# uta-smile/Adaptive-Graph-Convolutional-Network

Measured on NVIDIA B200. Metric: sgc_ll_train_graphs_per_s, higher is better.
Workload: dtype f32

## Files before the change

adaptive-graph-convolutional-network_b200/csrc/agcn_capi.cu:

```cuda
#include <algorithm>

#include "agcn_internal.cuh"

using namespace agcn;

namespace {

inline size_t align256(size_t x) { return (x + 255) & ~(size_t)255; }

int node_gemm_tn(const GemmTNArgs& t, cudaStream_t st) {
  if (tc_gemm_tn_supported(t)) return tc_gemm_tn(t, st);
  return gemm_tn(t, st);
}

int node_gemm(const GemmArgs& g, float* tc_scratch, cudaStream_t st, bool presplit = false) {
  if (tc_gemm_supported(g)) {
    if (!presplit) {
      int rc = tc_gemm_split_b(g, tc_scratch, st);
      if (rc) return rc;
    }
    return tc_gemm(g, tc_scratch, st);
  }
  return gemm_rows(g, st);
}
// ... 5 lines not shown
  g.A0 = X; g.lda0 = d->F;
  g.A1 = T; g.lda1 = d->F; g.sliceA1 = (int64_t)R * d->F;
  g.B = weight; g.ldb = d->K * d->Fo; g.sliceB = d->Fo;
  g.C = Y; g.ldc = d->Fo;
  g.bias = bias; g.act = d->activation;
  return g;
}

GemmArgs g_gemm_args(const agcn_sgcll_desc* d, int R, const float* dYp, const float* weight, float* C) {
  GemmArgs g;
  g.M = R; g.N = d->F; g.Kd = d->Fo; g.Z = d->K;
  g.A0 = dYp; g.lda0 = d->Fo;
  g.B = weight; g.ldb = d->K * d->Fo; g.sliceB = d->Fo; g.transB = 1;
  g.C = C; g.ldc = d->F; g.sliceC = (int64_t)R * d->F;
  return g;
}

struct Carver {
  char* base;
  size_t off = 0;
  explicit Carver(void* p) : base(reinterpret_cast<char*>(p)) {}
  float* take(size_t floats) {
    float* r = base ? reinterpret_cast<float*>(base + off) : nullptr;
    off += align256(floats * sizeof(float));
    return r;
  }
};

struct Modes {
  bool shortcut, paper, reslap, full, need_dL;
};

Modes modes_of(const agcn_sgcll_desc* d) {
  Modes m;
  m.shortcut = literal_shortcut(d->variant, d->laplacian_mode);
  m.paper = d->laplacian_mode == AGCN_LAP_PAPER;
  m.reslap = d->variant == AGCN_VARIANT_SGC_LL_RESLAP;
  m.full = m.paper && d->metric_grad == AGCN_METRIC_GRAD_FULL;
  m.need_dL = !m.shortcut;
  return m;
}

struct Saved {
  float *T, *Lall, *dist, *dis, *stats, *XW, *tcG, *ftG;
  size_t bytes;
};

Saved carve_saved(const agcn_sgcll_desc* d, const agcn_plan* p, void* base) {
  const Modes m = modes_of(d);
  Carver c(base);
  Saved s{};
  s.T = c.take((size_t)(d->K > 1 ? d->K - 1 : 0) * p->R * d->F);
  s.Lall = m.shortcut ? nullptr : c.take((size_t)p->LL);
  s.dist = m.paper ? c.take((size_t)p->LL) : nullptr;
  s.dis = m.paper ? c.take((size_t)p->R) : nullptr;
  s.stats = m.shortcut ? nullptr : c.take((size_t)4 * p->B);
  s.XW = m.full ? c.take((size_t)p->R * d->F) : nullptr;
  s.tcG = c.take(tc_gemm_scratch_floats(d->F, d->Fo, 1, d->K));
  s.ftG = c.take(fused_w_floats(d->F, d->Fo, d->K));
  s.bytes = c.off;
  return s;
}

inline int64_t dl_stride(const agcn_plan* p) { return (p->LL + 63) & ~(int64_t)63; }
inline int dl_parts(const agcn_sgcll_desc* d, const agcn_plan* p) {
  if (d->K < 2) return 1;
  int parts = std::min(8, (d->F + 31) / 32);
  while (parts > 1 && (int64_t)parts * dl_stride(p) * 4 > ((int64_t)1 << 30)) --parts;
  return std::max(1, parts);
}

struct Work {
  float *XW, *dYp, *G, *V, *tn_part, *act_part, *dL, *dXW, *dalpha_part, *dbeta_part, *tcY, *tcM, *big, *ftY;
  size_t bytes;
};

Work carve_work(const agcn_sgcll_desc* d, const agcn_plan* p, void* base) {
  const Modes m = modes_of(d);
  Carver c(base);
  Work w{};
  w.XW = c.take((size_t)p->R * d->F);
  w.dYp = c.take((size_t)p->R * d->Fo);
  w.G = c.take((size_t)d->K * p->R * d->F);
  w.V = c.take((size_t)(d->K > 1 ? d->K - 1 : 0) * p->R * d->Fo);
  size_t tn = gemm_tn_partial_floats((int)p->R, d->F, d->Fo, d->K);
  if (m.full) tn = std::max(tn, gemm_tn_partial_floats((int)p->R, d->F, d->F, 1));
  {
    GemmTNArgs t;
    t.M = (int)p->R; t.Kd = d->F; t.N = d->Fo; t.S = d->K;
    tn = std::max(tn, tc_gemm_tn_partial_floats(t));
    t.N = d->F; t.S = 1;
    tn = std::max(tn, tc_gemm_tn_partial_floats(t));
  }
  w.tn_part = c.take(tn);
  w.act_part = c.take(act_bwd_partial_floats(p->R, d->Fo));
  w.dL = m.need_dL ? c.take((size_t)dl_parts(d, p) * dl_stride(p)) : nullptr;
  w.dXW = m.full ? c.take((size_t)p->R * d->F) : nullptr;
  w.dalpha_part = c.take((size_t)p->B);
  w.dbeta_part = c.take((size_t)p->B);
  w.tcY = c.take(tc_gemm_scratch_floats(d->Fo, d->F, d->K, 1));
  w.tcM = c.take(tc_gemm_scratch_floats(d->F, d->F, 1, 1));
  w.big = c.take(big_work_floats(p, m.full));
  w.ftY = c.take(fused_w_floats(d->Fo, d->F, d->K));
  w.bytes = c.off;
  return w;
}

int check_desc(const agcn_sgcll_desc* d, const agcn_plan* p) {
  AGCN_REQUIRE(d && p, "null desc or plan");
  AGCN_REQUIRE(d->F >= 1 && d->Fo >= 1 && d->K >= 1, "F, Fo, K must be >= 1");
  AGCN_REQUIRE(d->variant == AGCN_VARIANT_SGC_LL || d->variant == AGCN_VARIANT_SGC_LL_RESLAP, "unknown variant");
  AGCN_REQUIRE(d->laplacian_mode == AGCN_LAP_REFERENCE_LITERAL || d->laplacian_mode == AGCN_LAP_PAPER,
               "unknown laplacian_mode");
  AGCN_REQUIRE(d->metric_grad == AGCN_METRIC_GRAD_REFERENCE || d->metric_grad == AGCN_METRIC_GRAD_FULL,
               "unknown metric_grad");
  AGCN_REQUIRE(d->activation == AGCN_ACT_LINEAR || d->activation == AGCN_ACT_RELU, "unknown activation");
  AGCN_REQUIRE(p->R < (1ll << 31) / std::max(d->F, d->Fo), "batch too large for 32-bit row indexing");
  return AGCN_OK;
}

}

namespace {

int padded_features(const agcn_sgcll_desc* d, const agcn_plan* p) {
  const int F = d->F;
  if (F < 33 || F % 32 == 0) return F;
  if (!literal_shortcut(d->variant, d->laplacian_mode)) return F;
  if (d->flags & (AGCN_OUT_RES_L | AGCN_OUT_RES_W | AGCN_OUT_L_ALL)) return F;
  const int Fp = (F + 31) & ~31;
  if (!fused_fwd_supported(p, Fp, d->Fo, d->K)) return F;
  return Fp;
}

struct PadSaved {
  float *Xp, *Wp;
  void* inner;
  size_t bytes;
};
PadSaved carve_pad_saved(const agcn_sgcll_desc* d2, const agcn_plan* p, void* base) {
  Carver c(base);
  PadSaved s{};
  s.Xp = c.take((size_t)p->R * d2->F);
  s.Wp = c.take((size_t)d2->F * d2->K * d2->Fo);
  s.inner = base ? reinterpret_cast<char*>(base) + c.off : nullptr;
  s.bytes = c.off + carve_saved(d2, p, nullptr).bytes + 256;
  return s;
}
struct PadWork {
  float *dXp, *dWp, *dMp;
  void* inner;
  size_t inner_bytes, bytes;
};
PadWork carve_pad_work(const agcn_sgcll_desc* d2, const agcn_plan* p, void* base) {
  Carver c(base);
  PadWork w{};
  w.dXp = c.take((size_t)p->R * d2->F);
  w.dWp = c.take((size_t)d2->F * d2->K * d2->Fo);
  w.dMp = c.take((size_t)d2->F * d2->F);
  w.inner = base ? reinterpret_cast<char*>(base) + c.off : nullptr;
  w.inner_bytes = carve_work(d2, p, nullptr).bytes + 256;
  w.bytes = c.off + w.inner_bytes;
  return w;
}

__global__ void pad_cols_kernel(const float* __restrict__ src, int Fs, float* __restrict__ dst, int Fd, long long rows) {
  const long long total = rows * Fd;
// ... 162 lines not shown
    AGCN_CUDA(cudaStreamWaitEvent(plan->side, plan->ev_side_fork, 0));
    if (fuse_f && (rc = fused_fwd_prep(d_weight, F, Fo, K, wk.ftY, plan->side))) return rc;
    if (y_tc && (rc = tc_gemm_split_b(gy, wk.tcY, plan->side))) return rc;
    if (fuse_b && (rc = fused_bwd_prep(d_weight, F, Fo, K, sv.ftG, plan->side))) return rc;
    if (g_tc && (rc = tc_gemm_split_b(gg, sv.tcG, plan->side))) return rc;
    AGCN_CUDA(cudaEventRecord(plan->ev_side_join, plan->side));
  }
  if (need_W) {
    GemmArgs g;
    g.M = R; g.N = F; g.Kd = F;
    g.A0 = d_X; g.lda0 = F;
    g.B = d_M_L; g.ldb = F;
    g.C = XW; g.ldc = F;
    if ((rc = node_gemm(g, wk.tcM, st))) return rc;
  }
  GraphArgs ga;
  ga.plan = plan; ga.F = F; ga.K = K;
  ga.variant = desc->variant; ga.lap_mode = desc->laplacian_mode; ga.metric_full = m.full;
  ga.X = d_X; ga.XW = XW; ga.Lint = d_Lint; ga.Lprev = m.reslap ? d_Lprev : nullptr;
  ga.alpha = d_alpha; ga.beta = d_beta;
  ga.T = sv.T;
  if (need_build) {
    ga.Lall = m.shortcut ? nullptr : sv.Lall;
    ga.Lall_out = want_Lall ? d_Lall : nullptr;
    ga.resL = want_resL ? d_resL : nullptr;
    ga.resW = want_resW ? d_resW : nullptr;
    ga.dist = sv.dist; ga.dis = sv.dis; ga.stats = sv.stats;
    ga.big_work = wk.big;
    if ((rc = graph_build_laplacian(ga, need_W, st))) return rc;
  }
  ga.Lall = m.shortcut ? nullptr : sv.Lall;
  if (fuse_f) {
    const float* Lf = m.shortcut ? d_Lint : sv.Lall;
    const int ident = m.shortcut ? 1 : 0;
    const bool other = cheb_tiles_has_mid(plan) || plan->large_tiles > 0;
    if (other) {
      AGCN_CUDA(cudaEventRecord(plan->ev_big_fork, st));
      AGCN_CUDA(cudaStreamWaitEvent(plan->big, plan->ev_big_fork, 0));
    }
    if ((rc = cheb_tiles_forward(plan, d_X, Lf, ident, F, K, sv.T, st, plan->big))) return rc;
    if (plan->large_tiles > 0 && (rc = graph_chebyshev_fwd(ga, plan->big, AGCN_SMALL_MAX))) return rc;
    if (other) {
      AGCN_CUDA(cudaEventRecord(plan->ev_big_join, plan->big));
      AGCN_CUDA(cudaStreamWaitEvent(st, plan->ev_big_join, 0));
    }
    AGCN_CUDA(cudaStreamWaitEvent(st, plan->ev_side_join, 0));
    return pre_forward(plan, -1, 0, d_X, sv.T, wk.ftY, d_bias, desc->activation, F, Fo, K, d_Y, st);
  }
  if ((rc = graph_chebyshev_fwd(ga, st))) return rc;
  if (y_tc || g_tc || fuse_b) AGCN_CUDA(cudaStreamWaitEvent(st, plan->ev_side_join, 0));
  if ((rc = node_gemm(gy, wk.tcY, st, true))) return rc;
  return AGCN_OK;
}

int backward_impl(const agcn_sgcll_desc* desc, const agcn_plan* plan, const float* d_X, const float* d_Lint,
                  const float* d_Lprev, const float* d_M_L, const float* d_weight, const float* d_alpha,
                  const float* d_beta, const float* d_Y, const float* d_dY, const float* d_dLall_in, const void* d_saved,
                  float* d_dX, float* d_dM_L, float* d_dweight, float* d_dbias, float* d_dalpha, float* d_dbeta,
                  float* d_dLprev, void* d_work, size_t work_bytes, void* stream) {
  int rc = check_desc(desc, plan);
  if (rc) return rc;
  AGCN_REQUIRE(d_X && d_Lint && d_M_L && d_weight && d_alpha && d_Y && d_dY && d_saved && d_work,
               "backward: null input pointer");
  AGCN_REQUIRE(d_dM_L && d_dweight && d_dbias && d_dalpha, "backward: null output pointer");
  const Modes m = modes_of(desc);
  AGCN_REQUIRE(!m.reslap || (d_beta && d_dbeta), "backward: beta / dbeta required for SGC_LL_Reslap");
  cudaStream_t st = (cudaStream_t)stream;
  if ((rc = plan_use(plan, st))) return rc;
  Saved sv = carve_saved(desc, plan, const_cast<void*>(d_saved));
  Work wk = carve_work(desc, plan, d_work);
  if (wk.bytes > work_bytes) {
    set_error("backward: workspace too small");
    return AGCN_ERR_WORKSPACE;
  }
  const int F = desc->F, Fo = desc->Fo, K = desc->K;
  const int R = (int)plan->R;
  const bool has_prev = m.reslap && d_Lprev;

  const bool fuse_b = (desc->flags & AGCN_SAVE_FOR_BACKWARD) && !m.need_dL && d_dX != nullptr &&
                      fused_bwd_supported(plan, F, Fo, K);
  const bool vfirst = fuse_b && plan->large_tiles == 0;
  const bool need_G = !fuse_b && (d_dX != nullptr || (m.need_dL && K >= 2));
  const float* dYp = (desc->activation == AGCN_ACT_RELU) ? wk.dYp : d_dY;
  const bool act_on_side = !vfirst && (fuse_b || (!need_G && !m.need_dL));
  if (!act_on_side && (rc = act_bwd_partials(d_dY, d_Y, wk.dYp, wk.act_part, R, Fo, desc->activation, st))) return rc;
  AGCN_CUDA(cudaEventRecord(plan->ev_side_fork, st));
  AGCN_CUDA(cudaStreamWaitEvent(plan->side, plan->ev_side_fork, 0));
  if (act_on_side && (rc = act_bwd_partials(d_dY, d_Y, wk.dYp, wk.act_part, R, Fo, desc->activation, plan->side)))
    return rc;
  if ((rc = act_bwd_reduce(wk.act_part, d_dbias, R, Fo, plan->side))) return rc;
  float* dXbuf = d_dX ? d_dX : wk.G;
  AGCN_REQUIRE(d_dX || !m.full, "backward: d_dX is required with metric_grad = full");
  if (need_G) {
    GemmArgs g = g_gemm_args(desc, R, dYp, d_weight, (K == 1) ? d_dX : wk.G);
    GemmArgs probe = g_gemm_args(desc, R, d_Y, d_weight, wk.G);
    const bool presplit = (desc->flags & AGCN_SAVE_FOR_BACKWARD) && tc_gemm_supported(probe);
    if ((rc = node_gemm(g, sv.tcG, st, presplit))) return rc;
  }
  GraphArgs ga;
  ga.plan = plan; ga.F = F; ga.K = K;
  ga.variant = desc->variant; ga.lap_mode = desc->laplacian_mode; ga.metric_full = m.full;
  ga.X = d_X; ga.XW = sv.XW; ga.Lint = d_Lint; ga.Lprev = has_prev ? d_Lprev : nullptr;
  ga.alpha = d_alpha; ga.beta = d_beta;
  ga.T = sv.T; ga.Lall = m.shortcut ? nullptr : sv.Lall;
  ga.dist = sv.dist; ga.dis = sv.dis; ga.stats = sv.stats;
  ga.G = wk.G; ga.dLall_in = d_dLall_in; ga.dX = dXbuf; ga.dL = wk.dL;
  ga.dl_parts = (m.need_dL && K >= 2) ? dl_parts(desc, plan) : 1;
  ga.dl_stride = dl_stride(plan);
  ga.dLprev = has_prev ? d_dLprev : nullptr;
  ga.dXW = wk.dXW; ga.dalpha_part = wk.dalpha_part; ga.dbeta_part = m.reslap ? wk.dbeta_part : nullptr;
  ga.big_work = wk.big;
  {
    GemmTNArgs t;
    t.M = R; t.Kd = F; t.N = Fo; t.S = K;
    t.A0 = d_X; t.lda0 = F;
    t.A1 = sv.T; t.lda1 = F; t.sliceA1 = (int64_t)R * F;
    t.D = dYp; t.ldd = Fo;
    t.out = d_dweight; t.partial = wk.tn_part;
    if ((rc = node_gemm_tn(t, plan->side))) return rc;
  }
  AGCN_CUDA(cudaEventRecord(plan->ev_side_join, plan->side));
  if (vfirst) {
    const float* Lf = m.shortcut ? d_Lint : sv.Lall;
    const int ident = m.shortcut ? 1 : 0;
    const bool other = cheb_tiles_has_mid(plan);
    if (other) {
      AGCN_CUDA(cudaEventRecord(plan->ev_big_fork, st));
      AGCN_CUDA(cudaStreamWaitEvent(plan->big, plan->ev_big_fork, 0));
    }
    if ((rc = cheb_tiles_forward(plan, dYp, Lf, ident, Fo, K, wk.V, st, plan->big, 1))) return rc;
    if (other) {
      AGCN_CUDA(cudaEventRecord(plan->ev_big_join, plan->big));
      AGCN_CUDA(cudaStreamWaitEvent(st, plan->ev_big_join, 0));
    }
    if ((rc = pre_forward(plan, -1, 0, dYp, wk.V, sv.ftG, nullptr, AGCN_ACT_LINEAR, Fo, F, K, d_dX, st))) return rc;
  } else if (fuse_b) {
    const float* Lf = m.shortcut ? d_Lint : sv.Lall;
    const int ident = m.shortcut ? 1 : 0;
    if ((rc = pre_backward(plan, -1, 0, d_dY, desc->activation == AGCN_ACT_RELU ? d_Y : nullptr, sv.ftG, F, Fo, K, wk.G, st)))
      return rc;
    const bool other = cheb_tiles_has_mid(plan) || plan->large_tiles > 0;
    if (other) {
      AGCN_CUDA(cudaEventRecord(plan->ev_big_fork, st));
      AGCN_CUDA(cudaStreamWaitEvent(plan->big, plan->ev_big_fork, 0));
    }
    if ((rc = cheb_tiles_backward(plan, wk.G, Lf, ident, F, K, d_dX, st, plan->big))) return rc;
    if (plan->large_tiles > 0 && (rc = graph_recurrence_bwd(ga, false, plan->big, AGCN_SMALL_MAX))) return rc;
    if (other) {
      AGCN_CUDA(cudaEventRecord(plan->ev_big_join, plan->big));
      AGCN_CUDA(cudaStreamWaitEvent(st, plan->ev_big_join, 0));
    }
  } else if (K >= 2) {
    if (need_G && (rc = graph_recurrence_bwd(ga, m.need_dL, st))) return rc;
  } else if (m.need_dL) {
    if (d_dLall_in)
      AGCN_CUDA(cudaMemcpyAsync(wk.dL, d_dLall_in, (size_t)plan->LL * sizeof(float), cudaMemcpyDeviceToDevice, st));
    else
      AGCN_CUDA(cudaMemsetAsync(wk.dL, 0, (size_t)plan->LL * sizeof(float), st));
  }
  AGCN_CUDA(cudaStreamWaitEvent(st, plan->ev_side_join, 0));
  if (m.need_dL) {
    if ((rc = graph_laplacian_bwd(ga, st))) return rc;
    if ((rc = reduce_scalar_parts(wk.dalpha_part, plan->B, d_dalpha, st))) return rc;
    if (m.reslap) {
      if ((rc = reduce_scalar_parts(wk.dbeta_part, plan->B, d_dbeta, st))) return rc;
    }
  } else {
    if ((rc = zero_async(d_dalpha, 1, st))) return rc;
  }
  if (m.full) {
    GemmTNArgs t;
    t.M = R; t.Kd = F; t.N = F; t.S = 1;
    t.A0 = d_X; t.lda0 = F;
    t.D = wk.dXW; t.ldd = F;
    t.out = d_dM_L; t.partial = wk.tn_part;
    if ((rc = node_gemm_tn(t, st))) return rc;
    GemmArgs g;
    g.M = R; g.N = F; g.Kd = F;
    g.A0 = wk.dXW; g.lda0 = F;
    g.B = d_M_L; g.ldb = F; g.transB = 1;
    g.C = d_dX; g.ldc = F; g.accumulate = 1;
    if ((rc = node_gemm(g, wk.tcM, st))) return rc;
  } else {
    if ((rc = zero_async(d_dM_L, (size_t)F * F, st))) return rc;
  }
  return AGCN_OK;
}

}

extern "C" {

size_t agcn_gemm_tn_scratch_bytes(int32_t M, int32_t Kd, int32_t N, int32_t S) {
  GemmTNArgs t;
  t.M = M; t.Kd = Kd; t.N = N; t.S = S;
  return 4 * std::max(gemm_tn_partial_floats(M, Kd, N, S), tc_gemm_tn_partial_floats(t)) + 256;
}

int agcn_gemm_tn(const float* d_A0, const float* d_A1, const float* d_D, float* d_out, int32_t M, int32_t Kd,
                 int32_t N, int32_t S, void* d_scratch, int32_t use_tensor_cores, void* stream) {
  AGCN_REQUIRE(d_A0 && d_D && d_out && d_scratch && M >= 1 && Kd >= 1 && N >= 1 && S >= 1, "gemm_tn: bad arguments");
  GemmTNArgs t;
  t.M = M; t.Kd = Kd; t.N = N; t.S = S;
  t.A0 = d_A0; t.lda0 = Kd;
  t.A1 = d_A1; t.lda1 = Kd; t.sliceA1 = (int64_t)M * Kd;
  t.D = d_D; t.ldd = N;
  t.out = d_out; t.partial = reinterpret_cast<float*>(d_scratch);
  if (use_tensor_cores) {
    if (!tc_gemm_tn_supported(t)) {
      set_error("gemm_tn: shape not supported by the tensor-core kernel");
      return AGCN_ERR_INVALID;
    }
    return tc_gemm_tn(t, (cudaStream_t)stream);
  }
  return gemm_tn(t, (cudaStream_t)stream);
}

size_t agcn_node_gemm_scratch_bytes(int32_t N, int32_t Kd) { return 4 * tc_gemm_scratch_floats(N, Kd, 1, 1) + 256; }

int agcn_node_gemm(const float* d_A, int32_t lda, const float* d_B, int32_t ldb, int32_t transB, float* d_C, int32_t ldc,
                   int32_t M, int32_t N, int32_t Kd, const float* d_bias, const float* d_scale, int32_t accumulate,
                   int32_t activation, void* d_scratch, void* stream) {
  AGCN_REQUIRE(d_A && d_B && d_C && d_scratch && M >= 1 && N >= 1 && Kd >= 1, "node_gemm: bad arguments");
  AGCN_REQUIRE(activation == AGCN_ACT_LINEAR || activation == AGCN_ACT_RELU, "node_gemm: unknown activation");
  GemmArgs g;
  g.M = M; g.N = N; g.Kd = Kd;
  g.A0 = d_A; g.lda0 = lda;
  g.B = d_B; g.ldb = ldb; g.transB = transB;
  g.C = d_C; g.ldc = ldc;
  g.bias = d_bias; g.scale = d_scale; g.accumulate = accumulate; g.act = activation;
  return node_gemm(g, reinterpret_cast<float*>(d_scratch), (cudaStream_t)stream);
}

int agcn_fused_profile(int enable) {
  fused_profile_enable(enable);
  return AGCN_OK;
}
int agcn_fused_profile_read(float* ms_sum, int* launches) { return fused_profile_read(ms_sum, launches); }

int agcn_fused_debug_set(void* d_buf) {
  fused_debug_set(d_buf);
  return AGCN_OK;
}

int agcn_sgcll_host_scratch_bytes(const agcn_sgcll_desc* desc, const agcn_plan* plan, size_t* bytes) {
  AGCN_REQUIRE(desc && plan && bytes, "null pointer");
  size_t saved = 0, work = 0;
  agcn_sgcll_workspace_bytes(desc, plan, &saved, &work);
  const size_t B = plan->B, N = plan->Nmax;
  size_t total = 0;
  total += align256(B * N * desc->F * 4) + align256(B * N * N * 4) + align256(B * N * desc->Fo * 4);
  total += align256((size_t)plan->R * desc->F * 4) + align256((size_t)plan->LL * 4) +
           align256((size_t)plan->R * desc->Fo * 4);
  total += align256(saved) + align256(work);
  *bytes = total;
  return AGCN_OK;
}

int agcn_sgcll_forward_host(const agcn_sgcll_desc* desc, const agcn_plan* plan, const float* h_X_padded,
                            const float* h_L_padded, const float* d_M_L, const float* d_weight, const float* d_bias,
                            const float* d_alpha, float* h_Y_padded, void* d_scratch, size_t scratch_bytes,
                            void* stream) {
  int rc = check_desc(desc, plan);
  if (rc) return rc;
  AGCN_REQUIRE(h_X_padded && h_L_padded && h_Y_padded && d_scratch, "forward_host: null pointer");
  AGCN_REQUIRE(desc->variant == AGCN_VARIANT_SGC_LL, "forward_host: SGC_LL only");
  AGCN_REQUIRE((desc->flags & (AGCN_OUT_RES_L | AGCN_OUT_RES_W | AGCN_OUT_L_ALL)) == 0,
// ... 54 lines not shown
```

adaptive-graph-convolutional-network_b200/csrc/agcn_cheb_tile.cu:

```cuda
#include <algorithm>
#include <mutex>

#include "agcn_internal.cuh"

namespace agcn {
namespace ct {

constexpr int CH = 32;
constexpr int CPITCH = 144;

__device__ __forceinline__ uint32_t smem_u32(const void* p) { return (uint32_t)__cvta_generic_to_shared(p); }
__device__ __forceinline__ float4 lds128(uint32_t a) {
  float4 v;
  asm volatile("ld.shared.v4.f32 {%0,%1,%2,%3}, [%4];\n" : "=f"(v.x), "=f"(v.y), "=f"(v.z), "=f"(v.w) : "r"(a) : "memory");
  return v;
}
__device__ __forceinline__ float lds32(uint32_t a) {
  float v;
  asm volatile("ld.shared.f32 %0, [%1];\n" : "=f"(v) : "r"(a) : "memory");
  return v;
}
__device__ __forceinline__ void sts128(uint32_t a, float4 v) {
  asm volatile("st.shared.v4.f32 [%0], {%1,%2,%3,%4};\n" ::"r"(a), "f"(v.x), "f"(v.y), "f"(v.z), "f"(v.w) : "memory");
}
__device__ __forceinline__ void sts32(uint32_t a, float v) {
  asm volatile("st.shared.f32 [%0], %1;\n" ::"r"(a), "f"(v) : "memory");
}
__device__ __forceinline__ void cp_async4(uint32_t sdst, const float* gsrc) {
  asm volatile("cp.async.ca.shared.global [%0], [%1], 4;\n" ::"r"(sdst), "l"(gsrc) : "memory");
}
__device__ __forceinline__ void cp_async16(uint32_t sdst, const float* gsrc) {
  asm volatile("cp.async.cg.shared.global [%0], [%1], 16;\n" ::"r"(sdst), "l"(gsrc) : "memory");
}
__device__ __forceinline__ void cp_async_commit() { asm volatile("cp.async.commit_group;\n" ::: "memory"); }
__device__ __forceinline__ void cp_async_wait_all() { asm volatile("cp.async.wait_group 0;\n" ::: "memory"); }

struct CtArgs {
  const int4* tile_graphs;
  const int32_t* tile_gstart;
  const int32_t* order;
  const int32_t* n_nodes;
  const int32_t* node_off;
  const int64_t* lap_off;
  int order_start;
  int chunks;
  int cpc;
  int groups;
  int rows;
  int lfloats;
  const float* L;
  int add_identity;
  int transL;
  int F, K;
  const float* X;
  float* T;
  long long tslice;
  const float* G;
  long long gslice;
  float* dX;
  unsigned long long* dbg;
};

#define CT_STAMP(slot)                                                                  \
  do {                                                                                  \
    if (p.dbg && threadIdx.x == 0) {                                                    \
      unsigned long long t__;                                                           \
      asm volatile("mov.u64 %0, %%globaltimer;\n" : "=l"(t__));                         \
      p.dbg[(long long)blockIdx.x * 128 + (slot)] = t__;                                \
    }                                                                                   \
  } while (0)

struct Row {
  int grow;
  int n;
  int r0;
  int lbase;
  int i;
  int pitch;
};

__device__ __forceinline__ void copy_matrix(const float* __restrict__ src, uint32_t dst, int n, int pitch) {
  const int warp = threadIdx.x >> 5, lane = threadIdx.x & 31, nw = blockDim.x >> 5;
  for (int i = warp; i < n; i += nw) {
    const float* srow = src + (long long)i * n;
    const uint32_t drow = dst + 4 * (i * pitch);
    for (int j = lane; j < n; j += 32) cp_async4(drow + 4 * j, srow + j);
  }
}

template <bool TILE>
__device__ __forceinline__ Row prologue(const CtArgs& p, int tile, int r, uint32_t s_glist, uint32_t sL) {
  Row t;
  t.grow = -1; t.n = 0; t.r0 = 0; t.lbase = 0; t.i = 0; t.pitch = 1;
  const int tid = threadIdx.x, nthreads = blockDim.x;
  if (TILE) {
    if (tid < 32) {
      int gs = 0, ge = 0;
      if (tid == 0) {
        gs = __ldg(p.tile_gstart + tile);
        ge = __ldg(p.tile_gstart + tile + 1);
      }
      gs = __shfl_sync(0xffffffffu, gs, 0);
      ge = __shfl_sync(0xffffffffu, ge, 0);
      const int ng2 = 2 * (ge - gs);
      for (int e = tid; e < ng2; e += 32) {
        const int4 v = __ldg(p.tile_graphs + 2 * gs + e);
        asm volatile("st.shared.v4.s32 [%0], {%1,%2,%3,%4};\n" ::"r"(s_glist + 16 * e), "r"(v.x), "r"(v.y), "r"(v.z), "r"(v.w) : "memory");
      }
      if (tid == 0) asm volatile("st.shared.s32 [%0], %1;\n" ::"r"(s_glist + 128 * 32), "r"(ge - gs) : "memory");
    }
    __syncthreads();
    int ng;
    asm volatile("ld.shared.s32 %0, [%1];\n" : "=r"(ng) : "r"(s_glist + 128 * 32) : "memory");
    for (int e = 0; e < ng; ++e) {
      int gx, gy, gz, gw, noff, lo, hi, pad;
      asm volatile("ld.shared.v4.s32 {%0,%1,%2,%3}, [%4];\n" : "=r"(gx), "=r"(gy), "=r"(gz), "=r"(gw) : "r"(s_glist + 32 * e) : "memory");
      asm volatile("ld.shared.v4.s32 {%0,%1,%2,%3}, [%4];\n" : "=r"(noff), "=r"(lo), "=r"(hi), "=r"(pad) : "r"(s_glist + 32 * e + 16) : "memory");
      if (r >= gy && r < gy + gz) {
        t.grow = noff + (r - gy);
        t.n = gz; t.r0 = gy; t.lbase = gw; t.i = r - gy; t.pitch = gz | 1;
      }
      const long long loff = (long long)(((unsigned long long)(unsigned)hi << 32) | (unsigned)lo);
      copy_matrix(p.L + loff, sL + 4 * gw, gz, gz | 1);
    }
  } else {
    const int g = p.order[p.order_start + tile];
    const int n = p.n_nodes[g], pitch = n | 1;
    if (r < n) {
      t.grow = p.node_off[g] + r;
      t.n = n; t.i = r; t.pitch = pitch;
    }
    copy_matrix(p.L + p.lap_off[g], sL, n, pitch);
  }
  cp_async_commit();
  return t;
}

// ... 65 lines not shown
}
template <int MW>
__device__ __forceinline__ void lap_times_rows_masked(uint32_t laddr, int lstride_bytes, uint32_t src, int r0,
                                                      const Mask<MW>& m, int h, float acc[16]) {
#pragma unroll
  for (int k = 0; k < MW; ++k) {
    uint32_t bits = m.w[k];
    const uint32_t tbase = src + (uint32_t)((r0 + 32 * k) * CPITCH + h * 64);
    const uint32_t lbase = laddr + (uint32_t)(32 * k * lstride_bytes);
    while (bits) {
      const int j = __ffs((int)bits) - 1;
      bits &= bits - 1;
      const float a = lds32(lbase + (uint32_t)(j * lstride_bytes));
      float4 b[4];
#pragma unroll
      for (int g = 0; g < 4; ++g) b[g] = lds128(tbase + (uint32_t)(j * CPITCH + 16 * g));
      fma_row(a, b, acc);
    }
  }
}

__device__ __forceinline__ uint32_t seg_addr(uint32_t buf, int row, int h) { return buf + (uint32_t)(row * CPITCH + h * 64); }
__device__ __forceinline__ void read_seg(uint32_t buf, int row, int h, float v[16]) {
#pragma unroll
  for (int g = 0; g < 4; ++g) {
    const float4 x = lds128(seg_addr(buf, row, h) + 16 * g);
    v[4 * g] = x.x; v[4 * g + 1] = x.y; v[4 * g + 2] = x.z; v[4 * g + 3] = x.w;
  }
}
__device__ __forceinline__ void write_seg(uint32_t buf, int row, int h, const float v[16]) {
#pragma unroll
  for (int g = 0; g < 4; ++g)
    sts128(seg_addr(buf, row, h) + 16 * g, make_float4(v[4 * g], v[4 * g + 1], v[4 * g + 2], v[4 * g + 3]));
}
__device__ __forceinline__ void load_seg(const float* __restrict__ M, int F, int grow, int col0, bool vec, float v[16]) {
  if (grow < 0) {
#pragma unroll
    for (int u = 0; u < 16; ++u) v[u] = 0.f;
    return;
  }
  const float* src = M + (long long)grow * F + col0;
  if (vec) {
#pragma unroll
    for (int g = 0; g < 4; ++g) {
      float4 x = make_float4(0.f, 0.f, 0.f, 0.f);
      if (col0 + 4 * g < F) x = __ldg(reinterpret_cast<const float4*>(src) + g);
      v[4 * g] = x.x; v[4 * g + 1] = x.y; v[4 * g + 2] = x.z; v[4 * g + 3] = x.w;
    }
  } else {
#pragma unroll
    for (int u = 0; u < 16; ++u) v[u] = (col0 + u < F) ? __ldg(src + u) : 0.f;
  }
}
__device__ __forceinline__ void store_seg(float* __restrict__ M, int F, int grow, int col0, bool vec, const float v[16]) {
  if (grow < 0) return;
  float* dst = M + (long long)grow * F + col0;
  if (vec) {
#pragma unroll
    for (int g = 0; g < 4; ++g)
      if (col0 + 4 * g < F)
        reinterpret_cast<float4*>(dst)[g] = make_float4(v[4 * g], v[4 * g + 1], v[4 * g + 2], v[4 * g + 3]);
  } else {
#pragma unroll
    for (int u = 0; u < 16; ++u)
      if (col0 + u < F) dst[u] = v[u];
  }
}

template <bool TILE, int MW>
__global__ void __launch_bounds__(TILE ? 256 : 320, TILE ? 3 : 1) cheb_tile_fwd_kernel(CtArgs p) {
  extern __shared__ __align__(16) uint8_t smem[];
  const uint32_t sbase = smem_u32(smem);
  const int rows = p.rows;
  const uint32_t buf0 = sbase, buf1 = sbase + (uint32_t)(rows * CPITCH), sL = buf1 + (uint32_t)(rows * CPITCH),
                 s_glist = sL + 4u * (uint32_t)p.lfloats;
  const int tile = blockIdx.x / p.groups, grp = blockIdx.x - tile * p.groups;
  const int warp = threadIdx.x >> 5, lane = threadIdx.x & 31, wpr = rows >> 5;
  const int h = warp / wpr, r = (warp - h * wpr) * 32 + lane;
  const int F = p.F, K = p.K;
  CT_STAMP(100);
  const Row me = prologue<TILE>(p, tile, r, s_glist, sL);
  CT_STAMP(101);
  const bool vec = ((F & 3) == 0) && ((reinterpret_cast<uintptr_t>(p.X) & 15) == 0) &&
                   ((reinterpret_cast<uintptr_t>(p.T) & 15) == 0) && ((p.tslice & 3) == 0);
  const uint32_t lrow = p.transL ? sL + 4 * (me.lbase + me.i) : sL + 4 * (me.lbase + me.i * me.pitch);
  const int lstep = p.transL ? 4 * me.pitch : 4;
  Mask<MW> mask;
  bool masked = false;
  const int c_beg = grp * p.cpc, c_end = min(p.chunks, c_beg + p.cpc);
  for (int c = c_beg; c < c_end; ++c) {
    const int col0 = c * CH + 16 * h;
    {
      const uint32_t d = seg_addr(buf0, r, h);
      const float* src = p.X + (long long)(me.grow < 0 ? 0 : me.grow) * F + col0;
      if (vec) {
#pragma unroll
        for (int g = 0; g < 4; ++g) {
          if (me.grow >= 0 && col0 + 4 * g < F)
            cp_async16(d + 16 * g, src + 4 * g);
          else
            sts128(d + 16 * g, make_float4(0.f, 0.f, 0.f, 0.f));
        }
      } else {
#pragma unroll
        for (int u = 0; u < 16; ++u) {
          if (me.grow >= 0 && col0 + u < F)
            cp_async4(d + 4 * u, src + u);
          else
            sts32(d + 4 * u, 0.f);
        }
      }
      cp_async_commit();
    }
    if (c == c_beg) CT_STAMP(102);
    cp_async_wait_all();
    __syncthreads();
    if (c == c_beg) {
      CT_STAMP(103);
      mask = nonzero_mask<MW>(lrow, lstep, me.n);
      masked = prefer_masked<MW>(mask, me.n);
      CT_STAMP(104);
    }
    float tm1[16], tm2[16];
    read_seg(buf0, r, h, tm1);
#pragma unroll
    for (int u = 0; u < 16; ++u) tm2[u] = 0.f;
    uint32_t src = buf0, dst = buf1;
    for (int s = 1; s < K; ++s) {
      float t[16];
#pragma unroll
      for (int u = 0; u < 16; ++u) t[u] = p.add_identity ? tm1[u] : 0.f;
      if (masked)
        lap_times_rows_masked<MW>(lrow, lstep, src, me.r0, mask, h, t);
      else
        lap_times_rows(lrow, lstep, src, me.r0, me.n, h, t);
      if (s >= 2) {
#pragma unroll
        for (int u = 0; u < 16; ++u) t[u] = 2.f * t[u] - tm2[u];
      }
      store_seg(p.T + (long long)(s - 1) * p.tslice, F, me.grow, col0, vec, t);
      if (s + 1 < K) {
        write_seg(dst, r, h, t);
        __syncthreads();
        const uint32_t tmp = src; src = dst; dst = tmp;
      }
#pragma unroll
      for (int u = 0; u < 16; ++u) { tm2[u] = tm1[u]; tm1[u] = t[u]; }
      if (c == c_beg) CT_STAMP(104 + s);
    }
    if (c + 1 < c_end) __syncthreads();
  }
}

template <bool TILE, int MW>
__global__ void __launch_bounds__(TILE ? 256 : 320, TILE ? 3 : 1) cheb_tile_bwd_kernel(CtArgs p) {
  extern __shared__ __align__(16) uint8_t smem[];
  const uint32_t sbase = smem_u32(smem);
  const int rows = p.rows;
  const uint32_t buf0 = sbase, buf1 = sbase + (uint32_t)(rows * CPITCH), sL = buf1 + (uint32_t)(rows * CPITCH),
                 s_glist = sL + 4u * (uint32_t)p.lfloats;
  const int tile = blockIdx.x / p.groups, grp = blockIdx.x - tile * p.groups;
  const int warp = threadIdx.x >> 5, lane = threadIdx.x & 31, wpr = rows >> 5;
  const int h = warp / wpr, r = (warp - h * wpr) * 32 + lane;
  const int F = p.F, K = p.K;
  const Row me = prologue<TILE>(p, tile, r, s_glist, sL);
  const bool vec = ((F & 3) == 0) && ((reinterpret_cast<uintptr_t>(p.G) & 15) == 0) &&
                   ((reinterpret_cast<uintptr_t>(p.dX) & 15) == 0) && ((p.gslice & 3) == 0);
  cp_async_wait_all();
  __syncthreads();
  const uint32_t lcol = sL + 4 * (me.lbase + me.i);
  const Mask<MW> mask = nonzero_mask<MW>(lcol, 4 * me.pitch, me.n);
  const bool masked = prefer_masked<MW>(mask, me.n);
  const uint32_t ub[2] = {buf0, buf1};
  const int c_beg = grp * p.cpc, c_end = min(p.chunks, c_beg + p.cpc);
  for (int c = c_beg; c < c_end; ++c) {
// ... 40 lines not shown
template <typename Kern>
static int opt_in(Kern k, size_t bytes) {
  cudaError_t e = cudaFuncSetAttribute(k, cudaFuncAttributeMaxDynamicSharedMemorySize, (int)bytes);
  if (e != cudaSuccess) return cuda_fail(e, "cudaFuncSetAttribute(cheb_tile)", __FILE__, __LINE__);
  return AGCN_OK;
}

static CtArgs base_args(const agcn_plan* plan, const float* L, int add_identity, int F, int K) {
  CtArgs a{};
  a.order = plan->d_order; a.n_nodes = plan->d_n; a.node_off = plan->d_node_off; a.lap_off = plan->d_lap_off;
  a.chunks = (F + CH - 1) / CH;
  a.L = L; a.add_identity = add_identity; a.F = F; a.K = K;
  a.dbg = g_dbg;
  return a;
}

static const Bucket* mid_bucket(const agcn_plan* plan) {
  for (const Bucket& b : plan->buckets)
    if (b.limit > AGCN_FUSE_MAX_N && b.max_n <= plan->cheb_small_max) return &b;
  return nullptr;
}

static int launch(const agcn_plan* plan, CtArgs a, bool forward, cudaStream_t st_small, cudaStream_t st_mid) {
  static std::once_flag once;
  static int once_rc = AGCN_OK;
  const size_t smem_tile = smem_bytes(128, AGCN_FUSE_LCAP, true);
  const int mid_rows = (AGCN_SMALL_MAX + 31) / 32 * 32;
  const size_t smem_mid = smem_bytes(mid_rows, AGCN_SMALL_MAX * (AGCN_SMALL_MAX | 1), false);
  std::call_once(once, [&] {
    int rc;
    if ((rc = opt_in(cheb_tile_fwd_kernel<true, 2>, smem_tile))) once_rc = rc;
    if ((rc = opt_in(cheb_tile_bwd_kernel<true, 2>, smem_tile))) once_rc = rc;
    if ((rc = opt_in(cheb_tile_fwd_kernel<false, 5>, smem_mid))) once_rc = rc;
    if ((rc = opt_in(cheb_tile_bwd_kernel<false, 5>, smem_mid))) once_rc = rc;
  });
  if (once_rc) return once_rc;
  if (const Bucket* b = mid_bucket(plan)) {
    CtArgs t = a;
    t.tile_graphs = nullptr;
    t.order_start = b->start;
    t.rows = mid_rows;
    t.lfloats = AGCN_SMALL_MAX * (AGCN_SMALL_MAX | 1);
    t.cpc = 1;
    t.groups = t.chunks;
    const unsigned grid = (unsigned)(b->count * t.chunks);
    {
      ProfScope prof(forward ? "ct::cheb_tile_fwd_kernel(mid)" : "ct::cheb_tile_bwd_kernel(mid)", st_mid);
      if (forward)
        cheb_tile_fwd_kernel<false, 5><<<grid, 2 * mid_rows, smem_mid, st_mid>>>(t);
      else
        cheb_tile_bwd_kernel<false, 5><<<grid, 2 * mid_rows, smem_mid, st_mid>>>(t);
    }
    AGCN_LAUNCH_CHECK();
  }
  if (plan->ft_small_tiles > 0) {
    CtArgs t = a;
    t.tile_graphs = reinterpret_cast<const int4*>(plan->d_ft_entries);
    t.tile_gstart = plan->d_ft_gstart;
    t.rows = 128;
    t.lfloats = AGCN_FUSE_LCAP;
    int sms = 148, dev = 0;
    if (cudaGetDevice(&dev) == cudaSuccess) cudaDeviceGetAttribute(&sms, cudaDevAttrMultiProcessorCount, dev);
    t.cpc = 1;
    while (t.cpc < t.chunks && plan->ft_small_tiles * ((t.chunks + t.cpc - 1) / t.cpc) > 3 * sms) ++t.cpc;
    t.groups = (t.chunks + t.cpc - 1) / t.cpc;
    const unsigned grid = (unsigned)(plan->ft_small_tiles * t.groups);
    ProfScope prof(forward ? "ct::cheb_tile_fwd_kernel" : "ct::cheb_tile_bwd_kernel", st_small);
    if (forward)
      cheb_tile_fwd_kernel<true, 2><<<grid, 256, smem_tile, st_small>>>(t);
    else
      cheb_tile_bwd_kernel<true, 2><<<grid, 256, smem_tile, st_small>>>(t);
  }
  if (plan->ft_small_tiles > 0) AGCN_LAUNCH_CHECK();
  return AGCN_OK;
}

}

void cheb_debug_set(void* d_buf) { ct::g_dbg = reinterpret_cast<unsigned long long*>(d_buf); }

bool cheb_tiles_has_mid(const agcn_plan* plan) { return ct::mid_bucket(plan) != nullptr; }

int cheb_tiles_forward(const agcn_plan* plan, const float* X, const float* L, int add_identity, int F, int K, float* T,
                       cudaStream_t st_small, cudaStream_t st_mid, int transL) {
  if (K < 2) return AGCN_OK;
  ct::CtArgs a = ct::base_args(plan, L, add_identity, F, K);
  a.transL = transL;
  a.X = X; a.T = T; a.tslice = (long long)plan->R * F;
  return ct::launch(plan, a, true, st_small, st_mid);
}

int cheb_tiles_backward(const agcn_plan* plan, const float* G, const float* L, int add_identity, int F, int K, float* dX,
                        cudaStream_t st_small, cudaStream_t st_mid) {
  if (K < 2) return AGCN_OK;
  ct::CtArgs a = ct::base_args(plan, L, add_identity, F, K);
  a.G = G; a.gslice = (long long)plan->R * F; a.dX = dX;
  return ct::launch(plan, a, false, st_small, st_mid);
}

}
```

adaptive-graph-convolutional-network_b200/csrc/agcn_internal.cuh:

```cuda
#pragma once
#include <cuda_runtime.h>
#include <stdint.h>

#include <atomic>
#include <string>
#include <vector>

#include "agcn_sgcll.h"

#define AGCN_SMALL_MAX 144
#define AGCN_CHEB_SMALL_MAX 144
#define AGCN_FUSE_MAX_N 64
#define AGCN_FUSE_LCAP 8320
#define AGCN_MID_TILED_MIN 32
#define AGCN_DEGREE_FLOOR 8.271806125530277e-25f

namespace agcn {

#ifdef __CUDACC__
__device__ __forceinline__ float tf32_rn(float x) {
  uint32_t r;
  asm("cvt.rna.tf32.f32 %0, %1;\n" : "=r"(r) : "f"(x));
  return __uint_as_float(r);
}
// ... 178 lines not shown
  const float* beta = nullptr;
  float* T = nullptr;
  float* Lall = nullptr;
  float* Lall_out = nullptr;
  float* resL = nullptr;
  float* resW = nullptr;
  float* dist = nullptr;
  float* dis = nullptr;
  float* stats = nullptr;
  const float* G = nullptr;
  const float* dLall_in = nullptr;
  float* dX = nullptr;
  float* dL = nullptr;
  int dl_parts = 1;
  int64_t dl_stride = 0;
  float* dLprev = nullptr;
  float* dXW = nullptr;
  float* dalpha_part = nullptr;
  float* dbeta_part = nullptr;
  float* big_work = nullptr;
};
bool literal_shortcut(int variant, int lap_mode);
int graph_build_laplacian(const GraphArgs& a, bool need_W, cudaStream_t st);
int graph_chebyshev_fwd(const GraphArgs& a, cudaStream_t st, int above_n = 0);
int graph_recurrence_bwd(const GraphArgs& a, bool need_dL, cudaStream_t st, int above_n = 0);
int graph_laplacian_bwd(const GraphArgs& a, cudaStream_t st);
int reduce_scalar_parts(const float* parts, int B, float* out, cudaStream_t st);
int large_chebyshev_fwd(const GraphArgs& a, cudaStream_t st);
int large_recurrence_bwd(const GraphArgs& a, float* G, bool big_only, cudaStream_t st);
size_t big_work_floats(const agcn_plan* plan, bool full);
int big_build_laplacian(const GraphArgs& a, bool need_W, float* big_work, cudaStream_t st);
int big_dL(const GraphArgs& a, const float* U, cudaStream_t st);
int big_laplacian_bwd(const GraphArgs& a, float* big_work, cudaStream_t st);

struct GroupedArgs {
  const int32_t* n_nodes;
  const int32_t* node_off;
  const int64_t* lap_off;
  const int32_t* tile_graph;
  const int32_t* tile_row;
  const float* L;
  int add_identity, transL;
  const float* In;
  const float* Sub;
  const float* Add;
  float* Out;
  float* Out2;
  float cmul;
  int F;
  const float* RowScale;
  const float* ScaleIn;
  unsigned long long* dbg;
  int force_uniform;
};
int grouped_launch(const agcn_plan* plan, int tiles, const GroupedArgs& g, cudaStream_t st);
int grouped_simt(int tiles, const GroupedArgs& g, cudaStream_t st);
bool grouped_tc_supported(const GroupedArgs& g);
int grouped_tc(const agcn_plan* plan, int tiles, const GroupedArgs& g, cudaStream_t st);
bool pair_tc_supported(const agcn_plan* plan, int F);
int pair_tc_similarity(const agcn_plan* plan, const float* XW, int F, float* norms, float* dist, float* resW, float* rowpart,
                       int ncb, cudaStream_t st);
int pair_tc_dL(const agcn_plan* plan, const float* U, const float* X, const float* T, int F, int K, const float* dL_in,
               float* dL, cudaStream_t st);
bool grouped_thin_supported(const GroupedArgs& g);
int grouped_thin(int tiles, const GroupedArgs& g, cudaStream_t st);

void fused_profile_enable(int on);
int fused_profile_read(float* ms_sum, int* launches);
void prof_enable(int on);
void fused_debug_set(void* d_buf);
bool fused_fwd_supported(const agcn_plan* plan, int F, int Fo, int K);
bool fused_bwd_supported(const agcn_plan* plan, int F, int Fo, int K);
size_t fused_w_floats(int Nv, int Kv, int Z);
int fused_fwd_prep(const float* weight, int F, int Fo, int K, float* scratch, cudaStream_t st);
int fused_bwd_prep(const float* weight, int F, int Fo, int K, float* scratch, cudaStream_t st);

int pre_forward(const agcn_plan* plan, int tile0, int ntiles, const float* X, const float* T, const float* wsplit,
                const float* bias, int act, int F, int Fo, int K, float* Y, cudaStream_t st);
int pre_backward(const agcn_plan* plan, int tile0, int ntiles, const float* dY, const float* Y, const float* wsplit, int F,
                 int Fo, int K, float* G, cudaStream_t st);

bool cheb_tiles_has_mid(const agcn_plan* plan);
int cheb_tiles_forward(const agcn_plan* plan, const float* X, const float* L, int add_identity, int F, int K, float* T,
                       cudaStream_t st_small, cudaStream_t st_mid, int transL = 0);
int cheb_tiles_backward(const agcn_plan* plan, const float* G, const float* L, int add_identity, int F, int K, float* dX,
                        cudaStream_t st_small, cudaStream_t st_mid);

class ProfScope {
 public:
  ProfScope(const char* name, cudaStream_t st);
  ~ProfScope();
  ProfScope(const ProfScope&) = delete;
  ProfScope& operator=(const ProfScope&) = delete;

 private:
  const char* name_;
  cudaStream_t st_;
  cudaEvent_t e0_;
};

int zero_async(float* dst, size_t floats, cudaStream_t st);
int plan_use(const agcn_plan* plan, cudaStream_t st);
int fork_streams(const agcn_plan* plan, cudaStream_t main, int n_aux);
int join_streams(const agcn_plan* plan, cudaStream_t main, int n_aux);

}
```

Before: 1.649 million.

## Fuse ReLU backward mask into Chebyshev tile forward and move zero-fills to side stream

In the V-first fused backward path, the ReLU derivative mask is now applied inside the Chebyshev tile forward kernel. The kernel reads dY and Y, writes the masked T0 slice into an enlarged V buffer, and uses it directly, so the separate activation-backward pass no longer runs on the main stream ahead of the tiles. The zero-fills of dalpha and dM_L move onto the side stream to overlap with the main stream's work. The cost is an extra Y read and T0 write inside the tile kernel, one more workspace slice, and extra alignment conditions before the vectorised path can be used.

```diff
diff --git a/adaptive-graph-convolutional-network_b200/csrc/agcn_capi.cu b/adaptive-graph-convolutional-network_b200/csrc/agcn_capi.cu
--- a/adaptive-graph-convolutional-network_b200/csrc/agcn_capi.cu
+++ b/adaptive-graph-convolutional-network_b200/csrc/agcn_capi.cu
@@ -111,7 +111,7 @@
   w.XW = c.take((size_t)p->R * d->F);
   w.dYp = c.take((size_t)p->R * d->Fo);
   w.G = c.take((size_t)d->K * p->R * d->F);
-  w.V = c.take((size_t)(d->K > 1 ? d->K - 1 : 0) * p->R * d->Fo);
+  w.V = c.take((size_t)(d->K > 1 ? d->K : 0) * p->R * d->Fo);
   size_t tn = gemm_tn_partial_floats((int)p->R, d->F, d->Fo, d->K);
   if (m.full) tn = std::max(tn, gemm_tn_partial_floats((int)p->R, d->F, d->F, 1));
   {
@@ -440,7 +440,7 @@
   const bool vfirst = fuse_b && plan->large_tiles == 0;
   const bool need_G = !fuse_b && (d_dX != nullptr || (m.need_dL && K >= 2));
   const float* dYp = (desc->activation == AGCN_ACT_RELU) ? wk.dYp : d_dY;
-  const bool act_on_side = !vfirst && (fuse_b || (!need_G && !m.need_dL));
+  const bool act_on_side = fuse_b || (!need_G && !m.need_dL);
   if (!act_on_side && (rc = act_bwd_partials(d_dY, d_Y, wk.dYp, wk.act_part, R, Fo, desc->activation, st))) return rc;
   AGCN_CUDA(cudaEventRecord(plan->ev_side_fork, st));
   AGCN_CUDA(cudaStreamWaitEvent(plan->side, plan->ev_side_fork, 0));
@@ -477,6 +477,8 @@
     t.out = d_dweight; t.partial = wk.tn_part;
     if ((rc = node_gemm_tn(t, plan->side))) return rc;
   }
+  if (!m.need_dL && (rc = zero_async(d_dalpha, 1, plan->side))) return rc;
+  if (!m.full && (rc = zero_async(d_dM_L, (size_t)F * F, plan->side))) return rc;
   AGCN_CUDA(cudaEventRecord(plan->ev_side_join, plan->side));
   if (vfirst) {
     const float* Lf = m.shortcut ? d_Lint : sv.Lall;
@@ -486,12 +488,18 @@
       AGCN_CUDA(cudaEventRecord(plan->ev_big_fork, st));
       AGCN_CUDA(cudaStreamWaitEvent(plan->big, plan->ev_big_fork, 0));
     }
-    if ((rc = cheb_tiles_forward(plan, dYp, Lf, ident, Fo, K, wk.V, st, plan->big, 1))) return rc;
+    const bool relu = desc->activation == AGCN_ACT_RELU;
+    float* V = wk.V + (size_t)R * Fo;
+    if ((rc = cheb_tiles_forward(plan, d_dY, Lf, ident, Fo, K, V, st, plan->big, 1, relu ? d_Y : nullptr,
+                                 relu ? wk.V : nullptr)))
+      return rc;
     if (other) {
       AGCN_CUDA(cudaEventRecord(plan->ev_big_join, plan->big));
       AGCN_CUDA(cudaStreamWaitEvent(st, plan->ev_big_join, 0));
     }
-    if ((rc = pre_forward(plan, -1, 0, dYp, wk.V, sv.ftG, nullptr, AGCN_ACT_LINEAR, Fo, F, K, d_dX, st))) return rc;
+    if ((rc = pre_forward(plan, -1, 0, relu ? wk.V : d_dY, V, sv.ftG, nullptr, AGCN_ACT_LINEAR, Fo, F, K, d_dX,
+                          st)))
+      return rc;
   } else if (fuse_b) {
     const float* Lf = m.shortcut ? d_Lint : sv.Lall;
     const int ident = m.shortcut ? 1 : 0;
@@ -523,8 +531,6 @@
     if (m.reslap) {
       if ((rc = reduce_scalar_parts(wk.dbeta_part, plan->B, d_dbeta, st))) return rc;
     }
-  } else {
-    if ((rc = zero_async(d_dalpha, 1, st))) return rc;
   }
   if (m.full) {
     GemmTNArgs t;
@@ -539,8 +545,6 @@
     g.B = d_M_L; g.ldb = F; g.transB = 1;
     g.C = d_dX; g.ldc = F; g.accumulate = 1;
     if ((rc = node_gemm(g, wk.tcM, st))) return rc;
-  } else {
-    if ((rc = zero_async(d_dM_L, (size_t)F * F, st))) return rc;
   }
   return AGCN_OK;
 }
diff --git a/adaptive-graph-convolutional-network_b200/csrc/agcn_cheb_tile.cu b/adaptive-graph-convolutional-network_b200/csrc/agcn_cheb_tile.cu
--- a/adaptive-graph-convolutional-network_b200/csrc/agcn_cheb_tile.cu
+++ b/adaptive-graph-convolutional-network_b200/csrc/agcn_cheb_tile.cu
@@ -53,6 +53,8 @@
   int transL;
   int F, K;
   const float* X;
+  const float* Ymask;
+  float* T0;
   float* T;
   long long tslice;
   const float* G;
@@ -284,7 +286,8 @@
   const Row me = prologue<TILE>(p, tile, r, s_glist, sL);
   CT_STAMP(101);
   const bool vec = ((F & 3) == 0) && ((reinterpret_cast<uintptr_t>(p.X) & 15) == 0) &&
-                   ((reinterpret_cast<uintptr_t>(p.T) & 15) == 0) && ((p.tslice & 3) == 0);
+                   ((reinterpret_cast<uintptr_t>(p.T) & 15) == 0) && ((p.tslice & 3) == 0) &&
+                   ((reinterpret_cast<uintptr_t>(p.Ymask) & 15) == 0) && ((reinterpret_cast<uintptr_t>(p.T0) & 15) == 0);
   const uint32_t lrow = p.transL ? sL + 4 * (me.lbase + me.i) : sL + 4 * (me.lbase + me.i * me.pitch);
   const int lstep = p.transL ? 4 * me.pitch : 4;
   Mask<MW> mask;
@@ -292,7 +295,15 @@
   const int c_beg = grp * p.cpc, c_end = min(p.chunks, c_beg + p.cpc);
   for (int c = c_beg; c < c_end; ++c) {
     const int col0 = c * CH + 16 * h;
-    {
+    if (p.Ymask) {
+      float v[16], m[16];
+      load_seg(p.X, F, me.grow, col0, vec, v);
+      load_seg(p.Ymask, F, me.grow, col0, vec, m);
+#pragma unroll
+      for (int u = 0; u < 16; ++u) v[u] = (m[u] > 0.f) ? v[u] : 0.f;
+      write_seg(buf0, r, h, v);
+      store_seg(p.T0, F, me.grow, col0, vec, v);
+    } else {
       const uint32_t d = seg_addr(buf0, r, h);
       const float* src = p.X + (long long)(me.grow < 0 ? 0 : me.grow) * F + col0;
       if (vec) {
@@ -499,10 +510,11 @@
 bool cheb_tiles_has_mid(const agcn_plan* plan) { return ct::mid_bucket(plan) != nullptr; }
 
 int cheb_tiles_forward(const agcn_plan* plan, const float* X, const float* L, int add_identity, int F, int K, float* T,
-                       cudaStream_t st_small, cudaStream_t st_mid, int transL) {
+                       cudaStream_t st_small, cudaStream_t st_mid, int transL, const float* Ymask, float* T0) {
   if (K < 2) return AGCN_OK;
   ct::CtArgs a = ct::base_args(plan, L, add_identity, F, K);
   a.transL = transL;
+  a.Ymask = Ymask; a.T0 = T0;
   a.X = X; a.T = T; a.tslice = (long long)plan->R * F;
   return ct::launch(plan, a, true, st_small, st_mid);
 }
diff --git a/adaptive-graph-convolutional-network_b200/csrc/agcn_internal.cuh b/adaptive-graph-convolutional-network_b200/csrc/agcn_internal.cuh
--- a/adaptive-graph-convolutional-network_b200/csrc/agcn_internal.cuh
+++ b/adaptive-graph-convolutional-network_b200/csrc/agcn_internal.cuh
@@ -284,7 +284,8 @@
 
 bool cheb_tiles_has_mid(const agcn_plan* plan);
 int cheb_tiles_forward(const agcn_plan* plan, const float* X, const float* L, int add_identity, int F, int K, float* T,
-                       cudaStream_t st_small, cudaStream_t st_mid, int transL = 0);
+                       cudaStream_t st_small, cudaStream_t st_mid, int transL = 0, const float* Ymask = nullptr,
+                       float* T0 = nullptr);
 int cheb_tiles_backward(const agcn_plan* plan, const float* G, const float* L, int add_identity, int F, int K, float* dX,
                         cudaStream_t st_small, cudaStream_t st_mid);
 
```

Result: slower. 1.628 million, median of 6 (-1.3%).
